# CycloneBoy/pdf_table

Hardware: AMD Instinct MI355X
Metric: pages/s (higher is better)
Workload: dtype bf16

## Files before the change

### include/pdftable_hip.h

```cpp
#ifndef PDFTABLE_HIP_H
#define PDFTABLE_HIP_H

#include <stddef.h>
#include <stdint.h>

#ifdef __cplusplus
extern "C" {
#endif

#define PT_OK 0
#define PT_ERR_INVALID 1
#define PT_ERR_HIP 2
#define PT_ERR_STATE 3
#define PT_ERR_FORMAT 4

typedef struct pt_engine pt_engine;
typedef void* pt_stream;

int pt_engine_create(int device_id, pt_engine** out);
void pt_engine_destroy(pt_engine* e);
const char* pt_last_error(void);
int pt_abi_version(void);
int pt_engine_check(pt_engine* e);
int pt_engine_set_lstm_cluster(pt_engine* e, int on);
// ... 162 lines not shown
                        const double* d_affine, int32_t* d_counts, float* d_cells, pt_stream stream);

int pt_tsr_process(pt_engine* e, const float* d_logi, const float* d_dets, const int32_t* h_counts, int n_tables,
                   int use_2dpe, float* d_logic, float* d_stacked, pt_stream stream);

int pt_op_conv2d(pt_engine* e, const uint16_t* d_in, int B, int H, int W, int Cin, const uint16_t* d_w_tiled,
                 const float* d_bias, int N, int ks, int stride, uint16_t* d_out, int out_cstride, int out_coff,
                 int rep, int shuffle_cout, const uint16_t* d_res, int res_mode, int relu, int split, int out_lo_off,
                 pt_stream stream);
int pt_op_conv1x1_ex(pt_engine* e, const uint16_t* d_in, int B, int H, int W, int Cin, const uint16_t* d_w_tiled, const float* d_bias,
                     int N, uint16_t* d_out, float* d_out_f32, int out_cstride, int n_valid, const float* d_res_f32, int relu,
                     const int32_t* d_ylimit, pt_stream stream);

int pt_op_dcn(pt_engine* e, const uint16_t* d_in, const float* d_om, int B, int H, int W, int C, const uint16_t* d_w_tiled,
              const float* d_bias, int N, uint16_t* d_out, int relu, int split, pt_stream stream);

int pt_op_stem7x7(pt_engine* e, const uint16_t* d_in, int B, int H, int W, const uint16_t* d_w, const float* d_bias,
                  uint16_t* d_out, int split, pt_stream stream);
int pt_op_maxpool3x3s2(pt_engine* e, const uint16_t* d_in, int B, int H, int W, int C, uint16_t* d_out, int split,
                       pt_stream stream);
int pt_op_db_head_final(pt_engine* e, const uint16_t* d_in, int B, int H, int W, const void* d_w, const float* d_bias,
                        float* d_prob, float* d_logits, int split, pt_stream stream);

int pt_op_dwconv(pt_engine* e, const uint16_t* d_in, int B, int H, int W, int C, const float* d_w_taps, const float* d_bias, int k,
                 int stride, int act, uint16_t* d_out, int split, pt_stream stream);
int pt_op_add(pt_engine* e, const uint16_t* d_a, const uint16_t* d_b, uint16_t* d_out, long long npix, int C, int split, pt_stream stream);
int pt_op_maxpool(pt_engine* e, const uint16_t* d_in, int B, int H, int W, int C, int k, int stride, int pad, uint16_t* d_out,
                  int split, pt_stream stream);
int pt_op_avgpool(pt_engine* e, const uint16_t* d_in, int B, int H, int W, int C, int k, uint16_t* d_out, int split, pt_stream stream);
int pt_op_chan_mean(pt_engine* e, const uint16_t* d_in, int B, int HW, int C, float* d_scratch, uint16_t* d_mean, int split, pt_stream stream);
// ... 90 lines not shown
```

### pdf_table_amd/csrc/c_api.hip

```cpp
#include <stdarg.h>
#include <stdio.h>
#include <stdlib.h>

#include <cmath>

#include "common.h"

namespace PT_FMT_NS {
namespace api {

static int ensure(void** buf, size_t* cap, size_t need);

int pt_engine_check(pt_engine* e) {
  PT_REQUIRE(e, "pt_engine_check: null engine");
  if (e->lstm_err && *e->lstm_err) {
    *e->lstm_err = 0;
    e->lstm_cluster = 0;
    pt_set_error("lstm_cluster_kernel: a workgroup waited > 2^22 polls for its peers -- the launch was not co-resident "
                 "(GPU shared with another process or stream?).  The recognition results since the last check are invalid; "
                 "this engine now uses the streaming LSTM kernel (pt_engine_set_lstm_cluster(e, 0)): run the batch again");
    return PT_ERR_HIP;
  }
  return PT_OK;
}
// ... 943 lines not shown
}

int pt_op_db_head_final(pt_engine* e, const uint16_t* d_in, int B, int H, int W, const void* d_w, const float* d_bias,
                        float* d_prob, float* d_logits, int split, pt_stream stream) {
  PT_REQUIRE(e && d_in && d_w && d_bias && (d_prob || d_logits), "pt_op_db_head_final: bad arguments");
  return pt_launch_db_head_final(d_in, B, H, W, d_w, d_bias, d_prob, d_logits, split, reinterpret_cast<hipStream_t>(stream));
}

int pt_op_dcn(pt_engine* e, const uint16_t* d_in, const float* d_om, int B, int H, int W, int C, const uint16_t* d_w_tiled,
              const float* d_bias, int N, uint16_t* d_out, int relu, int split, pt_stream stream) {
  PT_REQUIRE(e && d_in && d_om && d_w_tiled && d_bias && d_out, "pt_op_dcn: null argument");
  PT_REQUIRE(B > 0 && H > 0 && W > 0, "pt_op_dcn: empty map (B=%d H=%d W=%d)", B, H, W);
  return pt_launch_dcn_fused(e, d_in, d_om, d_w_tiled, d_bias, d_out, B, H, W, C, N, split, relu, reinterpret_cast<hipStream_t>(stream));
}

int pt_profile_enable(pt_engine* e, int on) {
  PT_REQUIRE(e != nullptr, "pt_profile_enable: null engine");
  PT_REQUIRE(on >= 0 && on < 2 + PT_PROF_NCLASS, "pt_profile_enable: mode %d out of range", on);
  if (on && !e->prof.h_lims)
    PT_HIP_CHECK(hipHostMalloc(reinterpret_cast<void**>(&e->prof.h_lims), PtProfile::MAX_LIMS * sizeof(int), hipHostMallocDefault));
  e->prof.on = on;
  return PT_OK;
}

int pt_profile_read_labels(pt_engine* e, char* buf, int cap) {
  PT_REQUIRE(e && buf && cap > 0, "pt_profile_read_labels: bad arguments");
  PT_HIP_CHECK(hipDeviceSynchronize());
  struct Row { double ms = 0, flop = 0, bytes = 0; long long n = 0; };
  std::map<std::string, Row> rows;
  for (auto& p : e->prof.pending) {
// ... 69 lines not shown
```

### pdf_table_amd/csrc/common.h

```cpp
#pragma once
#include <hip/hip_runtime.h>
#include <stdint.h>
#include <string.h>

#include <map>
#include <string>
#include <vector>

#include "../../include/pdftable_hip.h"
#include "act16.h"

typedef uint16_t bf16_t;

void pt_set_error(const char* fmt, ...);

#define PT_HIP_CHECK(expr)                                                                  \
  do {                                                                                      \
    hipError_t _e = (expr);                                                                 \
    if (_e != hipSuccess) {                                                                 \
      pt_set_error("%s failed: %s (%s:%d)", #expr, hipGetErrorString(_e), __FILE__, __LINE__); \
      return PT_ERR_HIP;                                                                    \
    }                                                                                       \
  } while (0)

// ... 219 lines not shown
  int alg_n = 0;
  double alg_scale = 1.0;
};
int pt_launch_conv(pt_engine* e, const ConvDesc& d, hipStream_t s);
int pt_launch_crnn_conv01(pt_engine* e, const bf16_t* gray, int n, const float* w64x9, const float* b0, const bf16_t* w1, const float* b1, bf16_t* p1,
                          const int* xlimit, const int* xlimit_cols, hipStream_t s);
int pt_launch_dwpw(pt_engine* e, const bf16_t* in, int B, int H, int W, int C, const float* dw_w, const float* dw_b, int k, int stride, int dw_act,
                   const ConvDesc& pw, hipStream_t s);

int pt_launch_stem7x7(pt_engine* e, const bf16_t* in, int B, int H, int W, const bf16_t* w, const float* bias,
                      bf16_t* out, int split, hipStream_t s, int stride = 2, int n_valid = 0);

int pt_launch_det_preprocess(const uint8_t* pages, int n, int h, int w, int nh, int nw, int flavour, int split,
                             bf16_t* out, hipStream_t s);
int pt_launch_dcn_fused(pt_engine* e, const bf16_t* x, const float* om, const bf16_t* w, const float* bias, bf16_t* out,
                        int B, int H, int W, int C, int N, int split, int relu, hipStream_t s, const bf16_t* omw = nullptr, const float* omb = nullptr);
bool pt_dcn_fuses_om(const pt_engine* e, int C, int split);
int pt_launch_maxpool3x3s2(const bf16_t* in, int B, int H, int W, int C, bf16_t* out, int split, hipStream_t s);
int pt_launch_stem7x7_pool(pt_engine* e, const bf16_t* in, int B, int H, int W, const bf16_t* w, const float* bias, bf16_t* out,
                           hipStream_t s);
int pt_launch_db_head_final(const bf16_t* in, int B, int H, int W, const void* w4x64, const float* bias, float* prob,
                            float* logits, int split, hipStream_t s);
int pt_launch_db_head_mfma(const bf16_t* in, int B, int H, int W, const bf16_t* w3, const float* b3, const bf16_t* w6,
                           const float* b6, float* prob, float* logits, hipStream_t s, uint32_t* bitmap = nullptr, float thresh = 0.f);
int pt_launch_bitmap(const float* prob, int n, int H, int W, float thresh, int dilate, uint32_t* bitmap,
                     hipStream_t s);
int pt_launch_box_scores(const float* prob, int n, int H, int W, const float* boxes, int nb, float* scores,
                         hipStream_t s);

#define PT_SE_CHUNKS 64
int pt_launch_stem3x3s2(const bf16_t* in, const float* w, const float* b, bf16_t* out, int B, int H, int W, int split,
                        hipStream_t s, int variant);
// ... 144 lines not shown
```

### pdf_table_amd/csrc/dla_net.h

```cpp
#pragma once

#include <stdlib.h>

#include <string>
#include <vector>

#include "net_ctx.h"

namespace PT_FMT_NS {

int pt_launch_conv3x3_c16(pt_engine* e, const bf16_t* in, const bf16_t* w, const float* bias, bf16_t* out, int B, int H, int W,
                          int N, int stride, int split, hipStream_t s);
int pt_launch_dla_thin_chain(pt_engine* e, const bf16_t* in, int B, int H, int W, const bf16_t* w_stem, const float* b_stem, const bf16_t* w0,
                             const float* b0, const bf16_t* w1, const float* b1, bf16_t* out, hipStream_t s);

namespace {

struct DlaCtx : NetCtx {
  bf16_t* cols = nullptr;
  float* om = nullptr;
  const int* ylimit = nullptr;
  double alg_scale = 1.0;

  void conv(const T& in, const std::string& q, int N, int ks, int stride, const T& out, int relu, const T* res = nullptr,
// ... 31 lines not shown
      e->prof.next_bytes = (double)n * x.H * x.W * x.C * 2.0 * mul * 1.25;
      PtProfScope ps(e, s, PT_PROF_OTHER, 0, "maxpool2x2");
      const int r = pt_launch_maxpool_kxk(x.p, n, x.H, x.W, x.C, 2, 2, 0, x3, o.p, s);
      if (r != PT_OK) rc = r;
    }
    return o;
  }
  T block(const std::string& q, const T& x, const T& residual, int stride, int cout) {
    T t = alloc(x.H / stride, x.W / stride, cout);
    conv(x, q + ".conv1", cout, 3, stride, t, 1);
    T o = alloc(t.H, t.W, cout);
    conv(t, q + ".conv2", cout, 3, 1, o, 1, &residual);
    return o;
  }
  T tree(const std::string& q, int levels, const T& x, int cin, int cout, int stride, bool level_root,
         std::vector<T> children) {
    T bottom = stride > 1 ? maxpool2(x) : x;
    if (level_root) children.push_back(bottom);
    if (levels == 1) {
      T residual = bottom;
      if (cin != cout) {
        residual = alloc(bottom.H, bottom.W, cout);
        conv(bottom, q + ".project", cout, 1, 1, residual, 0);
      }
      T x1 = block(q + ".tree1", x, residual, stride, cout);
      T x2 = block(q + ".tree2", x1, x1, 1, cout);
      std::vector<T> ins = {x2, x1};
      ins.insert(ins.end(), children.begin(), children.end());
      T o = alloc(x1.H, x1.W, cout);
      conv_cat(ins, q + ".root", cout, o, 1);
      return o;
    }
    T x1 = tree(q + ".tree1", levels - 1, x, cin, cout, stride, false, {});
    children.push_back(x1);
    return tree(q + ".tree2", levels - 1, x1, cout, cout, 1, false, children);
  }
};

static std::vector<T> dla34_base(DlaCtx& c, const bf16_t* x, int H, int W) {
  pt_engine* e = c.e;
  hipStream_t s = c.s;
  const int n = c.n;
  const int ch[6] = {16, 32, 64, 128, 256, 512};
  const int lv[6] = {1, 1, 1, 2, 2, 1};
  const char* chain_env = getenv("PT_DLA_CHAIN");
  const bool chain = !c.x3 && H % 2 == 0 && W % 2 == 0 && !(chain_env && atoi(chain_env) == 0);
  std::vector<T> layers(6);
  if (chain) {
// ... 37 lines not shown
```

### pdf_table_amd/csrc/lore_kernels.hip

```cpp
#include <stdio.h>
#include <stdlib.h>

#include "common.h"

namespace PT_FMT_NS {

typedef __attribute__((ext_vector_type(4))) uint32_t u32x4;
typedef __attribute__((ext_vector_type(2))) uint32_t u32x2;

namespace {

__device__ __forceinline__ float bf2f(uint32_t b) { return a16_to_f32(b); }
__device__ __forceinline__ uint32_t f2bf(float f) { return f32_to_a16(f); }

__device__ __forceinline__ void load8(const bf16_t* p, int lo_off, int split, float* v) {
  const u32x4 h = *reinterpret_cast<const u32x4*>(p);
  const uint32_t hw[4] = {h.x, h.y, h.z, h.w};
#pragma unroll
  for (int k = 0; k < 8; ++k) v[k] = bf2f((k & 1) ? (hw[k >> 1] >> 16) : (hw[k >> 1] & 0xFFFFu));
  if (split) {
    const u32x4 l = *reinterpret_cast<const u32x4*>(p + lo_off);
    const uint32_t lw[4] = {l.x, l.y, l.z, l.w};
#pragma unroll
    for (int k = 0; k < 8; ++k) v[k] += bf2f((k & 1) ? (lw[k >> 1] >> 16) : (lw[k >> 1] & 0xFFFFu));
// ... 451 lines not shown
    for (int r = 0; r < 16; ++r) {
      const long long op = p0 + wave * 32 + (r & 3) + 8 * (r >> 2) + 4 * q;
      if (op >= npix) continue;
      float v = acc[t][r] + bv;
      if (relu) v = fmaxf(v, 0.f);
      const uint32_t hb = f2bf(v);
      out[(size_t)op * ocs + n] = (bf16_t)hb;
      if (SPLIT) out[(size_t)op * ocs + N + n] = (bf16_t)f2bf(v - bf2f(hb));
    }
  }
}

#ifndef PT_DCN_ABL
#define PT_DCN_ABL 0
#endif
template <int NB, int NTHR, int SPLIT = 0, int EARLY = 0, int OMF = 0>
__global__ __launch_bounds__(NTHR, SPLIT ? (NB == 128 ? 1 : 2) : NTHR / 128) void dcn_fused64_kernel(const bf16_t* __restrict__ x, const float* __restrict__ om,
                                                              const bf16_t* __restrict__ w, const float* __restrict__ bias,
                                                              bf16_t* __restrict__ out, long long npix, int H, int W,
                                                              int C, int N, int relu, const bf16_t* __restrict__ omw = nullptr,
                                                              const float* __restrict__ omb = nullptr) {
#pragma clang fp contract(fast)
  a16_kernel_enter();
  constexpr int ROW = 144;
  constexpr int IT = 1024 / NTHR;
  constexpr int PSTEP = NTHR / 8;
  constexpr int WP = NB * 8 / NTHR;
  constexpr int NT = NB * 8 / NTHR;
  constexpr int NP = SPLIT ? 2 : 1;
  __shared__ __attribute__((aligned(16))) unsigned s_goff[128 * 9][4];
  __shared__ __attribute__((aligned(16))) float s_gwt[128 * 9][4];
  __shared__ __attribute__((aligned(16))) char s_ab[NP * (128 * ROW + NB * ROW)];
  static_assert(128 * ROW + NB * ROW >= 128 * 28 * 4, "operand images must cover the staged offset/mask rows");
  constexpr int A_PLANE = 128 * ROW, W_PLANE = NB * ROW;
  char* s_a = s_ab;
  char* s_w = s_ab + NP * A_PLANE;
  float* s_om = reinterpret_cast<float*>(s_ab);
// ... 7 lines not shown
  const int ty0 = (Lb % tiles_y) * 8;
  const long long img0 = (long long)(Lb / tiles_y) * H * W;
  auto locate = [&](int pl, int& y, int& xq) -> bool {
    y = ty0 + (pl >> 4);
    xq = tx0 + (pl & 15);
    const bool ok = y < H && xq < W;
    y = y < H ? y : H - 1;
    xq = xq < W ? xq : W - 1;
    return ok;
  };
  const int n0 = nblk * NB;
  const int nss = C >> 6, nst = 9 * nss, nk = 9 * (C >> 5);
  const int cs = SPLIT ? 2 * C : C;
  const int piece = tid & 7, prow = tid >> 3;
  const char* xmap = reinterpret_cast<const char*>(x + (size_t)img0 * cs);
  if constexpr (OMF) {
    constexpr int HP = 180, HROW = 80;
    constexpr int HIT = (HP * 4 + NTHR - 1) / NTHR;
    constexpr int NG = NTHR / 256;
    static_assert(sizeof(s_goff) >= HP * HROW && sizeof(s_gwt) >= HP * HROW, "a halo buffer must fit each table's space");
    char* s_h = reinterpret_cast<char*>(&s_goff[0][0]);
    char* s_h2 = reinterpret_cast<char*>(&s_gwt[0][0]);
    const int nch = (SPLIT ? 3 : 1) * (C >> 5);
    const int grp = wave >> 2, mt_o = wave & 3;
    const int t_lo = NG == 2 ? (grp ? 5 : 0) : 0, t_hi = NG == 2 ? (grp ? 9 : 5) : 9;
    u32x4 hreg[HIT];
    auto halo_load = [&](int kc) {
      int c0 = kc * 32;
      if (SPLIT && kc >= 2 * (C >> 5)) c0 -= 2 * C;
#pragma unroll
// ... 269 lines not shown
        }
      }
      __syncthreads();
      product();
    }
  } else {
    prefetch(0);
    for (int st = 0; st < nst; ++st) {
      __syncthreads();
      commit();
      __syncthreads();
      if (st + 1 < nst) prefetch(st + 1);
      product();
    }
  }
  int y, xq;
  if (locate(mt * 32 + lx, y, xq)) {
    bf16_t* op = out + (size_t)(img0 + (long long)y * W + xq) * (SPLIT ? 2 * N : N) + n0 + ct0 * 32;
#pragma unroll
    for (int t = 0; t < NT; ++t)
#pragma unroll
      for (int rg = 0; rg < 4; ++rg) {
        const int ch = t * 32 + 8 * rg + 4 * q;
        const float4 bs = *reinterpret_cast<const float4*>(bias + n0 + ct0 * 32 + ch);
        float v[4] = {acc[t][rg * 4 + 0] + bs.x, acc[t][rg * 4 + 1] + bs.y, acc[t][rg * 4 + 2] + bs.z, acc[t][rg * 4 + 3] + bs.w};
        if (relu) {
#pragma unroll
          for (int j = 0; j < 4; ++j) v[j] = fmaxf(v[j], 0.f);
        }
        const uint32_t h0 = f2bf(v[0]), h1 = f2bf(v[1]), h2 = f2bf(v[2]), h3 = f2bf(v[3]);
        *reinterpret_cast<uint2*>(op + ch) = make_uint2(h0 | (h1 << 16), h2 | (h3 << 16));
        if (SPLIT)
          *reinterpret_cast<uint2*>(op + N + ch) = make_uint2(f2bf(v[0] - bf2f(h0)) | (f2bf(v[1] - bf2f(h1)) << 16),
                                                               f2bf(v[2] - bf2f(h2)) | (f2bf(v[3] - bf2f(h3)) << 16));
      }
  }
}

#ifndef PT_DCN_MABL
#define PT_DCN_MABL 0
#endif
#ifndef PT_DCN_RING64
#define PT_DCN_RING64 4
#endif
template <int NB, int RING>
// ... 884 lines not shown
  PT_HIP_CHECK(hipGetLastError());
  return PT_OK;
}

bool pt_dcn_fuses_om(const pt_engine* e, int C, int split) {
  const char* ev = getenv("PT_DCN_FUSE_OM");
  const int on = ev ? atoi(ev) : 1;
  const char* nt = getenv("PT_DCN_THREADS");
  const char* ea = getenv("PT_DCN_EARLY");
  const char* xf = getenv("PT_DCN_X3_FAST");
  const bool defaults = !(nt && atoi(nt) != 512) && !(ea && atoi(ea) == 0) && !(xf && atoi(xf) == 0);
  if (!on || !e || C % 64 != 0 || !defaults || (!split && e->dcn_mfma != 0)) return false;
  return on == 2 || (!split && C <= 128);
}

int pt_launch_dcn_fused(pt_engine* e, const bf16_t* x, const float* om, const bf16_t* w, const float* bias, bf16_t* out,
                        int B, int H, int W, int C, int N, int split, int relu, hipStream_t s, const bf16_t* omw, const float* omb) {
  PT_REQUIRE(e && x && (om || (omw && omb)) && w && bias && out && C % 32 == 0 && N % 64 == 0, "dcn fused: bad arguments (C=%d N=%d)", C, N);
  PT_REQUIRE(!omw || pt_dcn_fuses_om(e, C, split), "dcn fused: the offset conv can only be fused on the default fused64 paths (C=%d)", C);
  PT_REQUIRE((long long)H * W * (split ? 2 * C : C) < (1ll << 31), "dcn fused: image too large for 32-bit offsets");
  const double dcn_bytes = (double)B * H * W * ((split ? 2.0 : 1.0) * 2.0 * (C + N) + 27 * 4.0) + (double)N * 9 * C * 2.0 * (split ? 3 : 1);
  e->prof.next_bytes = dcn_bytes;
  static int x3fast = -1;
  if (x3fast < 0) {
    const char* ev = getenv("PT_DCN_X3_FAST");
    x3fast = ev ? atoi(ev) : 1;
  }
  if (split && C % 64 == 0 && x3fast) {
    const long long npix = (long long)B * H * W;
    char label[48];
    snprintf(label, sizeof(label), "dcn fused %d->%d @%dx%d x3", C, N, H, W);
    PtProfScope prof(e, s, PT_PROF_OTHER, 0, label);
    const unsigned tiles = (unsigned)((long long)B * ((H + 7) / 8) * ((W + 15) / 16));
    const char* nbv = getenv("PT_DCN_NB");
    if (N % 128 == 0 && !(nbv && atoi(nbv) == 64)) {
      if (omw) hipLaunchKernelGGL((dcn_fused64_kernel<128, 512, 1, 0, 1>), dim3(tiles, N / 128), dim3(512), 0, s, x, om, w, bias, out, npix, H, W, C, N, relu, omw, omb);
      else hipLaunchKernelGGL((dcn_fused64_kernel<128, 512, 1>), dim3(tiles, N / 128), dim3(512), 0, s, x, om, w, bias, out, npix, H, W, C, N, relu, omw, omb);
    } else {
      if (omw) hipLaunchKernelGGL((dcn_fused64_kernel<64, 512, 1, 0, 1>), dim3(tiles, N / 64), dim3(512), 0, s, x, om, w, bias, out, npix, H, W, C, N, relu, omw, omb);
      else hipLaunchKernelGGL((dcn_fused64_kernel<64, 512, 1>), dim3(tiles, N / 64), dim3(512), 0, s, x, om, w, bias, out, npix, H, W, C, N, relu, omw, omb);
    }
    PT_HIP_CHECK(hipGetLastError());
    return PT_OK;
  }
  if (split) { e->prof.next_bytes = dcn_bytes; return launch_dcn_fused<1, 64>(e, x, om, w, bias, out, B, H, W, C, N, relu, s); }
  if (C % 64 == 0) {
    const long long npix = (long long)B * H * W;
    char label[48];
    snprintf(label, sizeof(label), "dcn fused %d->%d @%dx%d", C, N, H, W);
    PtProfScope prof(e, s, PT_PROF_OTHER, 0, label);
    static int nb128 = -1;
    if (nb128 < 0) {
      const char* ev = getenv("PT_DCN_NB");
      nb128 = ev ? (atoi(ev) == 128) : 1;
    }
    static int nthr = -1;
    if (nthr < 0) {
      const char* ev = getenv("PT_DCN_THREADS");
      nthr = ev ? atoi(ev) : 512;
    }
    const unsigned tiles = (unsigned)((long long)B * ((H + 7) / 8) * ((W + 15) / 16));
    static int mfma_nb = -1;
    if (mfma_nb < 0) {
      const char* nv = getenv("PT_DCN_MFMA_NB");
      PT_HIP_CHECK(hipFuncSetAttribute(reinterpret_cast<const void*>(&dcn_mfma_kernel<64, PT_DCN_RING64>), hipFuncAttributeMaxDynamicSharedMemorySize, DcnMfmaSmem<64, PT_DCN_RING64>::BYTES));
      PT_HIP_CHECK(hipFuncSetAttribute(reinterpret_cast<const void*>(&dcn_mfma_kernel<128, 8>), hipFuncAttributeMaxDynamicSharedMemorySize, DcnMfmaSmem<128, 8>::BYTES));
      mfma_nb = nv ? atoi(nv) : 128;
    }
    const int mfma = e->dcn_mfma;
    if (mfma == 2 && N == 64) {
      static bool attr2 = false;
      if (!attr2) {
        PT_HIP_CHECK(hipFuncSetAttribute(reinterpret_cast<const void*>(&dcn_mfma2_kernel), hipFuncAttributeMaxDynamicSharedMemorySize, DcnMfma2Smem::BYTES));
        attr2 = true;
      }
      const unsigned tiles2 = (unsigned)((long long)B * ((H + 15) / 16) * ((W + 15) / 16));
      hipLaunchKernelGGL(dcn_mfma2_kernel, dim3(tiles2, 1), dim3(512), DcnMfma2Smem::BYTES, s, x, om, w, bias, out, npix, H, W, C, N, relu);
      PT_HIP_CHECK(hipGetLastError());
      return PT_OK;
    }
    if (mfma == 1) {
      constexpr int smem64 = DcnMfmaSmem<64, PT_DCN_RING64>::BYTES, smem128 = DcnMfmaSmem<128, 8>::BYTES;
      if (N % 128 == 0 && mfma_nb == 128)
        hipLaunchKernelGGL((dcn_mfma_kernel<128, 8>), dim3(tiles, N / 128), dim3(512), smem128, s, x, om, w, bias, out, npix, H, W, C, N, relu);
// ... 79 lines not shown
```

### pdf_table_amd/csrc/lore_model.hip

```cpp
#include "dla_net.h"

namespace PT_FMT_NS {

int pt_launch_dcn_im2col(const bf16_t* x, const float* om, bf16_t* cols, int B, int H, int W, int C, int split,
                         hipStream_t s);
int pt_launch_dwconvt_up_add(const bf16_t* in, const float* w, const bf16_t* add, bf16_t* out, int B, int h, int wd,
                             int C, int f, int split, hipStream_t s);

namespace {

struct Ctx : DlaCtx {
  T dcn(const std::string& q, const T& x, int cout) {
    T o = alloc(x.H, x.W, cout);
    static const bool fused = !(getenv("PT_DCN_FUSED") && atoi(getenv("PT_DCN_FUSED")) == 0);
    const bool om_inside = fused && pt_dcn_fuses_om(e, x.C, x3);
    if (!om_inside) conv(x, q + ".om", 64, 3, 1, T(), 0, nullptr, 32, om, 32, 0, 27);
    if (fused) {
      const PtTensor* w = get(q + (x3 ? ".dcn.w3" : ".dcn.w"));
      const PtTensor* b = get(q + ".dcn.b");
      const PtTensor* ow = om_inside ? get(q + (x3 ? ".om.w3" : ".om.w")) : nullptr;
      const PtTensor* ob = om_inside ? get(q + ".om.b") : nullptr;
      if (go()) {
        const int r = pt_launch_dcn_fused(e, x.p, om, W(w), F(b), o.p, n, x.H, x.W, x.C, cout, x3, 1, s, ow ? W(ow) : nullptr, ob ? F(ob) : nullptr);
        if (r != PT_OK) rc = r;
      }
      return o;
    }
    if (go()) {
      PtProfScope ps(e, s, PT_PROF_OTHER, 0, "dcn im2col");
      const int r = pt_launch_dcn_im2col(x.p, om, cols, n, x.H, x.W, x.C, x3, s);
      if (r != PT_OK) rc = r;
    }
    T c;
    c.p = cols; c.H = x.H; c.W = x.W; c.C = 9 * x.C;
    conv(c, q + ".dcn", cout, 1, 1, o, 1);
    return o;
  }
  void ida(const std::string& q, std::vector<T>& layers, int startp, int endp, int o_ch, const int* up_f) {
    for (int i = startp + 1; i < endp; ++i) {
      const int j = i - startp;
      const std::string js = std::to_string(j);
      T p = dcn(q + ".proj_" + js, layers[i], o_ch);
      const int f = up_f[j];
      T u = alloc(p.H * f, p.W * f, o_ch);
      const PtTensor* wu = get(q + ".up_" + js + ".wf32");
      if (go()) {
        e->prof.next_bytes = (double)n * p.H * p.W * o_ch * 2.0 * mul * (1.0 + 2.0 * f * f);
        char label[48];
        snprintf(label, sizeof(label), "dw convT up + add %d @%dx%d", o_ch, p.H * f, p.W * f);
        PtProfScope ps(e, s, PT_PROF_OTHER, 0, label);
        const int r = pt_launch_dwconvt_up_add(p.p, F(wu), layers[i - 1].p, u.p, n, p.H, p.W, o_ch, f, x3, s);
        if (r != PT_OK) rc = r;
      }
      layers[i] = dcn(q + ".node_" + js, u, o_ch);
    }
  }
};

}

struct SparseArgs {
  int wiz_rev;
  float vis_thresh;
  int* d_counts;
  float *d_dets, *d_logi;
};

static int lore_dla_run(pt_engine* e, const bf16_t* x, int n, int H, int W, float* hm, float* st, float* wh, float* ax,
                        float* cr, float* reg, const SparseArgs* sp, hipStream_t s) {
// ... 9 lines not shown
  const int hreal[6] = {2, 8, 8, 256, 256, 2};

  return pt_plan_then_launch(c, "Lore net", [&]() -> int {
    const size_t px4 = (size_t)n * (H / 4) * (W / 4);
    c.cols = c.take<bf16_t>(px4 * 576 * c.mul * sizeof(bf16_t));
    c.om = c.take<float>(px4 * 32 * sizeof(float));

    std::vector<T> layers = dla34_base(c, x, H, W);

    std::vector<T> out = {layers[5]};
    const int f2[4] = {1, 2, 2, 2};
    c.ida("dla_up.ida_0", layers, 4, 6, 256, f2);
    out.insert(out.begin(), layers[5]);
    c.ida("dla_up.ida_1", layers, 3, 6, 128, f2);
    out.insert(out.begin(), layers[5]);
    c.ida("dla_up.ida_2", layers, 2, 6, 64, f2);
    out.insert(out.begin(), layers[5]);
    std::vector<T> y = {out[0], out[1], out[2]};
    const int f24[3] = {1, 2, 4};
    c.ida("ida_up", y, 0, 3, 64, f24);
    const T feat = y[2];
    T hid = c.alloc(feat.H, feat.W, 256);
    if (sp) heads[0] = c.take<float>((size_t)n * feat.H * feat.W * 8 * sizeof(float));
    for (int h = 0; h < 6; ++h) {
      if (sp && h != 0) continue;
      c.conv(feat, std::string(hname[h]) + ".0", 256, 3, 1, hid, 1);
      c.conv(hid, std::string(hname[h]) + ".2", hcs[h] < 64 ? 64 : hcs[h], 1, 1, T(), 0, nullptr, hcs[h], heads[h], hcs[h], 0, hreal[h]);
    }
    if (sp) {
      int rows_ax = 0, rows_cr = 0, rows_cell = 0, rows_corner = 0;
      pt_lore_mosaic_rows(n, &rows_ax, &rows_cr, &rows_cell, &rows_corner);
      const int MW = 32;
      auto mosaic = [&](int rows, int C) {
        T t;
        t.H = rows; t.W = MW; t.C = C;
// ... 153 lines not shown
```

### pdf_table_amd/engine.py

```python
from __future__ import annotations

import contextlib
import ctypes as C
import functools
import threading
from typing import Optional, Sequence, Tuple

import numpy as np
import torch

from . import lib as L

__all__ = ["HipEngine", "REC_LINE_DTYPE", "CLS_IMAGE_DTYPE", "REC_PP_ITEM_DTYPE"]

TSR_TABLE_DTYPE = np.dtype([("minv", "<f8", (6,)), ("page", "<i4"), ("x0", "<i4"), ("y0", "<i4"),
                            ("crop_w", "<i4"), ("crop_h", "<i4"), ("reserved", "<i4")])
CLS_IMAGE_DTYPE = np.dtype([("offset", "<i8"), ("h", "<i4"), ("w", "<i4")])
REC_LINE_DTYPE = np.dtype([("minv", np.float64, (9,)), ("page", np.int32), ("crop_w", np.int32), ("crop_h", np.int32),
                           ("reserved", np.int32)])


REC_PP_ITEM_DTYPE = np.dtype([("line", "<i4"), ("resized_w", "<i4"), ("img_w", "<i4"), ("reserved", "<i4"),
                              ("out_off", "<i8")])

# ... 629 lines not shown
    def op_dcn(self, x: torch.Tensor, om: torch.Tensor, w_tiled: torch.Tensor, bias: torch.Tensor, relu: bool = True, split: int = 0) -> torch.Tensor:
        self._chk(x, self.act_dtype, "x")
        self._chk(om, torch.float32, "om")
        self._chk(bias, torch.float32, "bias")
        B, H, W, Cc = x.shape
        m = 2 if split else 1
        Cc //= m
        if tuple(om.shape) != (B, H, W, 32):
            raise ValueError(f"op_dcn: om must be [B,H,W,32], got {tuple(om.shape)}")
        N = bias.numel()
        out = torch.empty((B, H, W, N * m), dtype=self.act_dtype, device=self._tdev)
        L.check(self.lib.pt_op_dcn(self._h, _ptr(x), _ptr(om), B, H, W, Cc, _ptr(w_tiled), _ptr(bias), N, _ptr(out), int(relu), int(split),
                                   self._stream()), "pt_op_dcn")
        return out

    def op_dwconv(self, x: torch.Tensor, w_taps: torch.Tensor, bias: torch.Tensor, k: int, stride: int = 1, act: int = 0, split: bool = False) -> torch.Tensor:
        self._chk(x, self.act_dtype, "x")
        self._chk(w_taps, torch.float32, "w_taps")
        self._chk(bias, torch.float32, "bias")
        B, H, W, Cc = x.shape
        pad = k // 2
        out = torch.empty((B, (H + 2 * pad - k) // stride + 1, (W + 2 * pad - k) // stride + 1, Cc), dtype=self.act_dtype, device=self._tdev)
        L.check(self.lib.pt_op_dwconv(self._h, _ptr(x), B, H, W, Cc // 2 if split else Cc, _ptr(w_taps), _ptr(bias), k, stride, act, _ptr(out), int(split),
                                      self._stream()), "pt_op_dwconv")
        return out

    def op_add(self, a: torch.Tensor, b: torch.Tensor, split: bool = False) -> torch.Tensor:
        self._chk(a, self.act_dtype, "a")
        self._chk(b, self.act_dtype, "b")
        if a.shape != b.shape:
# ... 332 lines not shown
```

### pdf_table_amd/lib.py

```python
from __future__ import annotations

import ctypes as C
import os

_HERE = os.path.dirname(os.path.abspath(__file__))
LIB_PATH = os.environ.get("PT_LIB_PATH") or os.path.join(_HERE, "libpdftable_hip.so")

PT_MODEL_DB_RESNET18 = 1
PT_MODEL_CRNN = 2
PT_MODEL_LORE_DLA34 = 3
PT_MODEL_LORE_PROCESSOR = 4
PT_MODEL_PICODET = 5
PT_MODEL_LORE_RESNET18 = 6
PT_MODEL_DB_NAS = 7
PT_MODEL_PPLCNET = 8
PT_MODEL_CONVNEXT_VIT = 16
PT_MODEL_MTL_BACKBONE = 17
PT_MODEL_MTL_DECODER = 18
PT_MODEL_CENTERNET_DLA34 = 19
PT_CVIT_W, PT_CVIT_CHUNK_W, PT_CVIT_CHUNK_STEP, PT_CVIT_T, PT_CVIT_NCLS = 804, 300, 252, 201, 7644
PT_CLS_SLOTS = 4
PT_CLS_MAX_CLASSES = 16
PT_LAYOUT_HEAD_CS, PT_LAYOUT_CAND_FLOATS = 40, 48
PT_DET_PRE_DB_PP = 0
# ... 75 lines not shown
        "pt_centernet_decode": (i, [vp, vp, vp, vp, vp, i, i, i, vp, vp, vp, vp]),
        "pt_hard_nms": (i, [vp, vp, vp, i, C.c_double, i, vp, vp]),
        "pt_page_line_mask": (i, [vp, i, i, i, vp, vp]),
        "pt_page_line_angles": (i, [vp, i, i, i, i, i, vp, i, vp]),
        "pt_page_warp_cubic": (i, [vp, i, i, i, vp, vp, i, vp, vp]),
        "pt_page_quarter_turn": (i, [vp, i, i, i, i, vp, vp]),
        "pt_page_pre_tables": (i, [vp, vp]),
        "pt_cls_preprocess": (i, [vp, vp, vp, i, i, i, i, i, vp, vp]),
        "pt_cls_forward_net": (i, [vp, i, vp, i, i, i, i, vp, ip, vp]),
        "pt_cls_forward": (i, [vp, i, vp, vp, i, i, i, i, i, i, vp, ip, vp]),
        "pt_cls_forward_lines": (i, [vp, i, vp, i, i, i, vp, vp, i, i, i, i, i, i, vp, ip, vp]),
        "pt_cls_forward_lines_direct": (i, [vp, i, vp, i, i, i, vp, i, i, i, i, i, i, vp, ip, vp]),
        "pt_op_conv2d": (i, [vp, vp, i, i, i, i, vp, vp, i, i, i, vp, i, i, i, i, vp, i, i, i, i, vp]),
        "pt_op_conv1x1_ex": (i, [vp, vp, i, i, i, i, vp, vp, i, vp, vp, i, i, vp, i, vp, vp]),
        "pt_op_dcn": (i, [vp, vp, vp, i, i, i, i, vp, vp, i, vp, i, i, vp]),
        "pt_op_stem7x7": (i, [vp, vp, i, i, i, vp, vp, vp, i, vp]),
        "pt_op_maxpool3x3s2": (i, [vp, vp, i, i, i, i, vp, i, vp]),
        "pt_op_db_head_final": (i, [vp, vp, i, i, i, vp, vp, vp, vp, i, vp]),
        "pt_op_dwconv": (i, [vp, vp, i, i, i, i, vp, vp, i, i, i, vp, i, vp]),
        "pt_op_add": (i, [vp, vp, vp, vp, C.c_longlong, i, i, vp]),
        "pt_op_maxpool": (i, [vp, vp, i, i, i, i, i, i, i, vp, i, vp]),
        "pt_op_avgpool": (i, [vp, vp, i, i, i, i, i, vp, i, vp]),
        "pt_op_chan_mean": (i, [vp, vp, i, i, i, vp, vp, i, vp]),
        "pt_op_chan_mean_scratch_floats": (i, [i, i]),
        "pt_op_scale_channels": (i, [vp, vp, vp, i, i, i, vp, i, vp]),
        "pt_op_act": (i, [vp, vp, C.c_longlong, i, C.c_float, C.c_float, vp, i, i, vp]),
        "pt_op_copy_channels": (i, [vp, vp, C.c_longlong, i, i, vp, i, i, i, vp]),
        "pt_op_upsample_nearest": (i, [vp, vp, i, i, i, i, i, vp, vp]),
        "pt_op_mul": (i, [vp, vp, vp, vp, C.c_longlong, i, i, vp]),
        "pt_copy_bytes": (i, [vp, vp, vp, C.c_longlong, vp]),
# ... 49 lines not shown
```

Before: 804.4.

## Fuse depthwise transposed-conv upsample+add into DCN node epilogue; pool once in DLA tree

Adds an epilogue to the fused DCN kernel that stages the low-resolution projection patch and the transposed-conv taps in dead shared buffers. The kernel then computes the 2x/4x depthwise upsample and adds it to the node output, so the separate dwconvT up+add launch and its full-resolution read and write go away. The IDA aggregation is reordered so each node's DCN emits the next level's upsampled sum directly. The change also reuses the pooled input in DLA tree recursion instead of max-pooling twice. It costs extra shared memory, registers and epilogue work in the DCN kernel, and is limited to the default single-pass configurations.

```diff
diff --git a/include/pdftable_hip.h b/include/pdftable_hip.h
--- a/include/pdftable_hip.h
+++ b/include/pdftable_hip.h
@@ -200,6 +200,12 @@
 
 int pt_op_dcn(pt_engine* e, const uint16_t* d_in, const float* d_om, int B, int H, int W, int C, const uint16_t* d_w_tiled,
               const float* d_bias, int N, uint16_t* d_out, int relu, int split, pt_stream stream);
+
+int pt_op_dwconvt_up_add(pt_engine* e, const uint16_t* d_in, const float* d_w, const uint16_t* d_add, uint16_t* d_out, int B, int h, int w, int C,
+                         int f, int split, pt_stream stream);
+int pt_op_dcn_up_add(pt_engine* e, const uint16_t* d_in, const float* d_om, int B, int H, int W, int C, const uint16_t* d_w_tiled,
+                     const float* d_bias, int N, uint16_t* d_out, int relu, int split, const uint16_t* d_up_in, int up_h, int up_w,
+                     const float* d_up_w, int up_f, pt_stream stream);
 
 int pt_op_stem7x7(pt_engine* e, const uint16_t* d_in, int B, int H, int W, const uint16_t* d_w, const float* d_bias,
                   uint16_t* d_out, int split, pt_stream stream);
diff --git a/pdf_table_amd/csrc/c_api.hip b/pdf_table_amd/csrc/c_api.hip
--- a/pdf_table_amd/csrc/c_api.hip
+++ b/pdf_table_amd/csrc/c_api.hip
@@ -981,6 +981,25 @@
   return pt_launch_dcn_fused(e, d_in, d_om, d_w_tiled, d_bias, d_out, B, H, W, C, N, split, relu, reinterpret_cast<hipStream_t>(stream));
 }
 
+int pt_op_dwconvt_up_add(pt_engine* e, const uint16_t* d_in, const float* d_w, const uint16_t* d_add, uint16_t* d_out, int B, int h, int w, int C,
+                         int f, int split, pt_stream stream) {
+  PT_REQUIRE(e && d_in && d_w && d_out, "pt_op_dwconvt_up_add: null argument");
+  PT_REQUIRE(B > 0 && h > 0 && w > 0 && C > 0, "pt_op_dwconvt_up_add: empty map (B=%d h=%d w=%d C=%d)", B, h, w, C);
+  return pt_launch_dwconvt_up_add(d_in, d_w, d_add, d_out, B, h, w, C, f, split, reinterpret_cast<hipStream_t>(stream));
+}
+
+int pt_op_dcn_up_add(pt_engine* e, const uint16_t* d_in, const float* d_om, int B, int H, int W, int C, const uint16_t* d_w_tiled,
+                     const float* d_bias, int N, uint16_t* d_out, int relu, int split, const uint16_t* d_up_in, int up_h, int up_w,
+                     const float* d_up_w, int up_f, pt_stream stream) {
+  PT_REQUIRE(e && d_in && d_om && d_w_tiled && d_bias && d_out && d_up_in && d_up_w, "pt_op_dcn_up_add: null argument");
+  PT_REQUIRE(B > 0 && H > 0 && W > 0, "pt_op_dcn_up_add: empty map (B=%d H=%d W=%d)", B, H, W);
+  PT_REQUIRE(split == 0, "pt_op_dcn_up_add: the (hi | lo) modes keep the two launches (pt_op_dcn, pt_op_dwconvt_up_add)");
+  PT_REQUIRE((up_f == 2 || up_f == 4) && up_h > 0 && up_w > 0 && up_h * up_f == H && up_w * up_f == W,
+             "pt_op_dcn_up_add: a %dx%d map times %d is not the %dx%d output", up_h, up_w, up_f, H, W);
+  return pt_launch_dcn_fused(e, d_in, d_om, d_w_tiled, d_bias, d_out, B, H, W, C, N, split, relu, reinterpret_cast<hipStream_t>(stream), nullptr, nullptr,
+                             d_up_in, d_up_w, up_f);
+}
+
 int pt_profile_enable(pt_engine* e, int on) {
   PT_REQUIRE(e != nullptr, "pt_profile_enable: null engine");
   PT_REQUIRE(on >= 0 && on < 2 + PT_PROF_NCLASS, "pt_profile_enable: mode %d out of range", on);
diff --git a/pdf_table_amd/csrc/common.h b/pdf_table_amd/csrc/common.h
--- a/pdf_table_amd/csrc/common.h
+++ b/pdf_table_amd/csrc/common.h
@@ -257,8 +257,12 @@
 int pt_launch_det_preprocess(const uint8_t* pages, int n, int h, int w, int nh, int nw, int flavour, int split,
                              bf16_t* out, hipStream_t s);
 int pt_launch_dcn_fused(pt_engine* e, const bf16_t* x, const float* om, const bf16_t* w, const float* bias, bf16_t* out,
-                        int B, int H, int W, int C, int N, int split, int relu, hipStream_t s, const bf16_t* omw = nullptr, const float* omb = nullptr);
+                        int B, int H, int W, int C, int N, int split, int relu, hipStream_t s, const bf16_t* omw = nullptr, const float* omb = nullptr,
+                        const bf16_t* up_in = nullptr, const float* up_w = nullptr, int up_f = 0);
 bool pt_dcn_fuses_om(const pt_engine* e, int C, int split);
+bool pt_dcn_fuses_up(const pt_engine* e, int C, int N, int split);
+int pt_launch_dwconvt_up_add(const bf16_t* in, const float* w, const bf16_t* add, bf16_t* out, int B, int h, int wd, int C, int f, int split,
+                             hipStream_t s);
 int pt_launch_maxpool3x3s2(const bf16_t* in, int B, int H, int W, int C, bf16_t* out, int split, hipStream_t s);
 int pt_launch_stem7x7_pool(pt_engine* e, const bf16_t* in, int B, int H, int W, const bf16_t* w, const float* bias, bf16_t* out,
                            hipStream_t s);
diff --git a/pdf_table_amd/csrc/dla_net.h b/pdf_table_amd/csrc/dla_net.h
--- a/pdf_table_amd/csrc/dla_net.h
+++ b/pdf_table_amd/csrc/dla_net.h
@@ -69,8 +69,8 @@
     return o;
   }
   T tree(const std::string& q, int levels, const T& x, int cin, int cout, int stride, bool level_root,
-         std::vector<T> children) {
-    T bottom = stride > 1 ? maxpool2(x) : x;
+         std::vector<T> children, const T* pooled = nullptr) {
+    T bottom = stride > 1 ? (pooled ? *pooled : maxpool2(x)) : x;
     if (level_root) children.push_back(bottom);
     if (levels == 1) {
       T residual = bottom;
@@ -86,7 +86,9 @@
       conv_cat(ins, q + ".root", cout, o, 1);
       return o;
     }
-    T x1 = tree(q + ".tree1", levels - 1, x, cin, cout, stride, false, {});
+    const char* once_env = getenv("PT_DLA_POOL_ONCE");
+    const bool once = stride > 1 && !(once_env && atoi(once_env) == 0);
+    T x1 = tree(q + ".tree1", levels - 1, x, cin, cout, stride, false, {}, once ? &bottom : nullptr);
     children.push_back(x1);
     return tree(q + ".tree2", levels - 1, x1, cout, cout, 1, false, children);
   }
diff --git a/pdf_table_amd/csrc/lore_kernels.hip b/pdf_table_amd/csrc/lore_kernels.hip
--- a/pdf_table_amd/csrc/lore_kernels.hip
+++ b/pdf_table_amd/csrc/lore_kernels.hip
@@ -489,13 +489,17 @@
 #ifndef PT_DCN_ABL
 #define PT_DCN_ABL 0
 #endif
-template <int NB, int NTHR, int SPLIT = 0, int EARLY = 0, int OMF = 0>
+__device__ __forceinline__ float dcn_up_mad(float acc, float v, float wt) { return acc + v * wt; }
+
+template <int NB, int NTHR, int SPLIT = 0, int EARLY = 0, int OMF = 0, int UPF = 0>
 __global__ __launch_bounds__(NTHR, SPLIT ? (NB == 128 ? 1 : 2) : NTHR / 128) void dcn_fused64_kernel(const bf16_t* __restrict__ x, const float* __restrict__ om,
                                                               const bf16_t* __restrict__ w, const float* __restrict__ bias,
                                                               bf16_t* __restrict__ out, long long npix, int H, int W,
                                                               int C, int N, int relu, const bf16_t* __restrict__ omw = nullptr,
-                                                              const float* __restrict__ omb = nullptr) {
+                                                              const float* __restrict__ omb = nullptr, const bf16_t* __restrict__ up_in = nullptr,
+                                                              const float* __restrict__ up_w = nullptr) {
 #pragma clang fp contract(fast)
+  static_assert(UPF == 0 || ((UPF == 2 || UPF == 4) && !SPLIT), "the up-sampling epilogue exists for factors 2 and 4 of the single-pass modes");
   a16_kernel_enter();
   constexpr int ROW = 144;
   constexpr int IT = 1024 / NTHR;
@@ -533,6 +537,25 @@
   const int cs = SPLIT ? 2 * C : C;
   const int piece = tid & 7, prow = tid >> 3;
   const char* xmap = reinterpret_cast<const char*>(x + (size_t)img0 * cs);
+  constexpr int UPH = UPF ? 8 / UPF + 2 : 1, UPW = UPF ? 16 / UPF + 2 : 1;
+  constexpr int UPITCH = NB * 2 + 16, WPITCH = NB + 8;
+  constexpr int UPP = UPF ? (UPH * UPW * (NB / 8) + NTHR - 1) / NTHR : 1;
+  constexpr int UPWT = UPF ? (4 * UPF * UPF * (NB / 4) + NTHR - 1) / NTHR : 1;
+  [[maybe_unused]] u32x4 upreg[UPP];
+  if constexpr (UPF != 0) {
+    static_assert(UPH * UPW * UPITCH <= (int)sizeof(s_ab) && 4 * UPF * UPF * WPITCH * 4 <= (int)sizeof(s_gwt), "the staged patch and table must fit the dead buffers");
+    const int uh = H / UPF, uw = W / UPF;
+    const long long ub = (img0 / ((long long)H * W)) * uh;
+#pragma unroll
+    for (int j = 0; j < UPP; ++j) {
+      const int i = tid + j * NTHR, pp = i / (NB / 8), pc = i - pp * (NB / 8);
+      const int r = pp / UPW, c = pp - r * UPW;
+      const int iy = min(max(ty0 / UPF - 1 + r, 0), uh - 1), ix = min(max(tx0 / UPF - 1 + c, 0), uw - 1);
+      u32x4 v = {0u, 0u, 0u, 0u};
+      if (i < UPH * UPW * (NB / 8)) v = *reinterpret_cast<const u32x4*>(up_in + (size_t)((ub + iy) * uw + ix) * N + n0 + pc * 8);
+      upreg[j] = v;
+    }
+  }
   if constexpr (OMF) {
     constexpr int HP = 180, HROW = 80;
     constexpr int HIT = (HP * 4 + NTHR - 1) / NTHR;
@@ -832,9 +855,49 @@
       product();
     }
   }
+  if constexpr (UPF != 0) {
+    float4 wreg[UPWT];
+#pragma unroll
+    for (int j = 0; j < UPWT; ++j) {
+      const int i = tid + j * NTHR;
+      float4 v = make_float4(0.f, 0.f, 0.f, 0.f);
+      if (i < 4 * UPF * UPF * (NB / 4)) v = *reinterpret_cast<const float4*>(up_w + (size_t)(i / (NB / 4)) * N + n0 + (i % (NB / 4)) * 4);
+      wreg[j] = v;
+    }
+    __syncthreads();
+#pragma unroll
+    for (int j = 0; j < UPP; ++j) {
+      const int i = tid + j * NTHR, pp = i / (NB / 8), pc = i - pp * (NB / 8);
+      if (i < UPH * UPW * (NB / 8)) *reinterpret_cast<u32x4*>(s_ab + pp * UPITCH + pc * 16) = upreg[j];
+    }
+#pragma unroll
+    for (int j = 0; j < UPWT; ++j) {
+      const int i = tid + j * NTHR;
+      if (i < 4 * UPF * UPF * (NB / 4)) *reinterpret_cast<float4*>(reinterpret_cast<float*>(&s_gwt[0][0]) + (i / (NB / 4)) * WPITCH + (i % (NB / 4)) * 4) = wreg[j];
+    }
+    __syncthreads();
+  }
   int y, xq;
   if (locate(mt * 32 + lx, y, xq)) {
     bf16_t* op = out + (size_t)(img0 + (long long)y * W + xq) * (SPLIT ? 2 * N : N) + n0 + ct0 * 32;
+    [[maybe_unused]] const char* up_p[2][2];
+    [[maybe_unused]] const float* up_t[2][2];
+    [[maybe_unused]] bool up_ok[2][2];
+    if constexpr (UPF != 0) {
+      const int uh = H / UPF, uw = W / UPF;
+      const int iy1 = (y + UPF / 2) / UPF, ix1 = (xq + UPF / 2) / UPF;
+#pragma unroll
+      for (int dy = 0; dy < 2; ++dy)
+#pragma unroll
+        for (int dx = 0; dx < 2; ++dx) {
+          const int iy = iy1 - dy, ix = ix1 - dx;
+          const int ky = y + UPF / 2 - iy * UPF, kx = xq + UPF / 2 - ix * UPF;
+          up_ok[dy][dx] = iy >= 0 && iy < uh && ix >= 0 && ix < uw;
+          const int iyc = min(max(iy, 0), uh - 1), ixc = min(max(ix, 0), uw - 1);
+          up_p[dy][dx] = s_ab + ((iyc - (ty0 / UPF - 1)) * UPW + (ixc - (tx0 / UPF - 1))) * UPITCH + ct0 * 64;
+          up_t[dy][dx] = reinterpret_cast<const float*>(&s_gwt[0][0]) + (ky * (2 * UPF) + kx) * WPITCH + ct0 * 32;
+        }
+    }
 #pragma unroll
     for (int t = 0; t < NT; ++t)
 #pragma unroll
@@ -846,7 +909,24 @@
 #pragma unroll
           for (int j = 0; j < 4; ++j) v[j] = fmaxf(v[j], 0.f);
         }
-        const uint32_t h0 = f2bf(v[0]), h1 = f2bf(v[1]), h2 = f2bf(v[2]), h3 = f2bf(v[3]);
+        uint32_t h0 = f2bf(v[0]), h1 = f2bf(v[1]), h2 = f2bf(v[2]), h3 = f2bf(v[3]);
+        if constexpr (UPF != 0) {
+          float us[4] = {0.f, 0.f, 0.f, 0.f};
+#pragma unroll
+          for (int dy = 0; dy < 2; ++dy)
+#pragma unroll
+            for (int dx = 0; dx < 2; ++dx) {
+              if (UPF == 4 && !up_ok[dy][dx]) continue;
+              uint2 pv = *reinterpret_cast<const uint2*>(up_p[dy][dx] + ch * 2);
+              if (UPF == 2 && !up_ok[dy][dx]) pv = make_uint2(0u, 0u);
+              const float4 wv = *reinterpret_cast<const float4*>(up_t[dy][dx] + ch);
+              us[0] = dcn_up_mad(us[0], bf2f(pv.x & 0xFFFFu), wv.x);
+              us[1] = dcn_up_mad(us[1], bf2f(pv.x >> 16), wv.y);
+              us[2] = dcn_up_mad(us[2], bf2f(pv.y & 0xFFFFu), wv.z);
+              us[3] = dcn_up_mad(us[3], bf2f(pv.y >> 16), wv.w);
+            }
+          h0 = f2bf(us[0] + bf2f(h0)); h1 = f2bf(us[1] + bf2f(h1)); h2 = f2bf(us[2] + bf2f(h2)); h3 = f2bf(us[3] + bf2f(h3));
+        }
         *reinterpret_cast<uint2*>(op + ch) = make_uint2(h0 | (h1 << 16), h2 | (h3 << 16));
         if (SPLIT)
           *reinterpret_cast<uint2*>(op + N + ch) = make_uint2(f2bf(v[0] - bf2f(h0)) | (f2bf(v[1] - bf2f(h1)) << 16),
@@ -1761,12 +1841,27 @@
   return on == 2 || (!split && C <= 128);
 }
 
+bool pt_dcn_fuses_up(const pt_engine* e, int C, int N, int split) {
+  const char* ev = getenv("PT_IDA_FUSE_UP");
+  if ((ev && atoi(ev) == 0) || !e || split || e->dcn_mfma != 0 || C != N || (N != 64 && N != 128)) return false;
+  for (const char* name : {"PT_DCN_FUSED", "PT_DCN_FUSE_OM", "PT_DCN_THREADS", "PT_DCN_EARLY", "PT_DCN_NB", "PT_DCN_MFMA", "PT_DCN_MFMA_NB", "PT_DCN_X3_FAST"})
+    if (getenv(name)) return false;
+  return true;
+}
+
 int pt_launch_dcn_fused(pt_engine* e, const bf16_t* x, const float* om, const bf16_t* w, const float* bias, bf16_t* out,
-                        int B, int H, int W, int C, int N, int split, int relu, hipStream_t s, const bf16_t* omw, const float* omb) {
+                        int B, int H, int W, int C, int N, int split, int relu, hipStream_t s, const bf16_t* omw, const float* omb,
+                        const bf16_t* up_in, const float* up_w, int up_f) {
   PT_REQUIRE(e && x && (om || (omw && omb)) && w && bias && out && C % 32 == 0 && N % 64 == 0, "dcn fused: bad arguments (C=%d N=%d)", C, N);
   PT_REQUIRE(!omw || pt_dcn_fuses_om(e, C, split), "dcn fused: the offset conv can only be fused on the default fused64 paths (C=%d)", C);
   PT_REQUIRE((long long)H * W * (split ? 2 * C : C) < (1ll << 31), "dcn fused: image too large for 32-bit offsets");
-  const double dcn_bytes = (double)B * H * W * ((split ? 2.0 : 1.0) * 2.0 * (C + N) + 27 * 4.0) + (double)N * 9 * C * 2.0 * (split ? 3 : 1);
+  if (up_f) {
+    PT_REQUIRE(up_in && up_w && (up_f == 2 || (up_f == 4 && N == 64)) && H % up_f == 0 && W % up_f == 0,
+               "dcn fused + up: factor %d must be 2 (or 4 at 64 channels) and divide the %dx%d map", up_f, H, W);
+    PT_REQUIRE(pt_dcn_fuses_up(e, C, N, split), "dcn fused + up: only the default single-pass kernels at C = N = 64 or 128 carry the up-sampling epilogue (C=%d N=%d split=%d)", C, N, split);
+  }
+  const double dcn_bytes = (double)B * H * W * ((split ? 2.0 : 1.0) * 2.0 * (C + N) + 27 * 4.0) + (double)N * 9 * C * 2.0 * (split ? 3 : 1) +
+                           (up_f ? (double)B * (H / up_f) * (W / up_f) * N * 2.0 : 0.0);
   e->prof.next_bytes = dcn_bytes;
   static int x3fast = -1;
   if (x3fast < 0) {
@@ -1794,7 +1889,7 @@
   if (C % 64 == 0) {
     const long long npix = (long long)B * H * W;
     char label[48];
-    snprintf(label, sizeof(label), "dcn fused %d->%d @%dx%d", C, N, H, W);
+    snprintf(label, sizeof(label), "dcn fused%s %d->%d @%dx%d", up_f ? "+up" : "", C, N, H, W);
     PtProfScope prof(e, s, PT_PROF_OTHER, 0, label);
     static int nb128 = -1;
     if (nb128 < 0) {
@@ -1815,6 +1910,18 @@
       mfma_nb = nv ? atoi(nv) : 128;
     }
     const int mfma = e->dcn_mfma;
+    if (up_f) {
+      const unsigned blk = N == 128 ? 256 : 512;
+#define PT_DCN_UP(NB_, NT_, EARLY_, OMF_, UPF_)                                                                                                   \
+  hipLaunchKernelGGL((dcn_fused64_kernel<NB_, NT_, 0, EARLY_, OMF_, UPF_>), dim3(tiles, N / NB_), dim3(blk), 0, s, x, om, w, bias, out, npix, H, W, C, N, relu, \
+                     omw, omb, up_in, up_w)
+      if (N == 128) { if (omw) PT_DCN_UP(128, 256, 0, 1, 2); else PT_DCN_UP(128, 256, 0, 0, 2); }
+      else if (up_f == 2) { if (omw) PT_DCN_UP(64, 512, 1, 1, 2); else PT_DCN_UP(64, 512, 1, 0, 2); }
+      else { if (omw) PT_DCN_UP(64, 512, 1, 1, 4); else PT_DCN_UP(64, 512, 1, 0, 4); }
+#undef PT_DCN_UP
+      PT_HIP_CHECK(hipGetLastError());
+      return PT_OK;
+    }
     if (mfma == 2 && N == 64) {
       static bool attr2 = false;
       if (!attr2) {
diff --git a/pdf_table_amd/csrc/lore_model.hip b/pdf_table_amd/csrc/lore_model.hip
--- a/pdf_table_amd/csrc/lore_model.hip
+++ b/pdf_table_amd/csrc/lore_model.hip
@@ -4,13 +4,15 @@
 
 int pt_launch_dcn_im2col(const bf16_t* x, const float* om, bf16_t* cols, int B, int H, int W, int C, int split,
                          hipStream_t s);
-int pt_launch_dwconvt_up_add(const bf16_t* in, const float* w, const bf16_t* add, bf16_t* out, int B, int h, int wd,
-                             int C, int f, int split, hipStream_t s);
-
 namespace {
 
 struct Ctx : DlaCtx {
-  T dcn(const std::string& q, const T& x, int cout) {
+  struct UpTail {
+    T p;
+    const PtTensor* w = nullptr;
+    int f = 0;
+  };
+  T dcn(const std::string& q, const T& x, int cout, const UpTail* up = nullptr) {
     T o = alloc(x.H, x.W, cout);
     static const bool fused = !(getenv("PT_DCN_FUSED") && atoi(getenv("PT_DCN_FUSED")) == 0);
     const bool om_inside = fused && pt_dcn_fuses_om(e, x.C, x3);
@@ -21,7 +23,8 @@
       const PtTensor* ow = om_inside ? get(q + (x3 ? ".om.w3" : ".om.w")) : nullptr;
       const PtTensor* ob = om_inside ? get(q + ".om.b") : nullptr;
       if (go()) {
-        const int r = pt_launch_dcn_fused(e, x.p, om, W(w), F(b), o.p, n, x.H, x.W, x.C, cout, x3, 1, s, ow ? W(ow) : nullptr, ob ? F(ob) : nullptr);
+        const int r = pt_launch_dcn_fused(e, x.p, om, W(w), F(b), o.p, n, x.H, x.W, x.C, cout, x3, 1, s, ow ? W(ow) : nullptr, ob ? F(ob) : nullptr,
+                                          up ? up->p.p : nullptr, up ? F(up->w) : nullptr, up ? up->f : 0);
         if (r != PT_OK) rc = r;
       }
       return o;
@@ -36,23 +39,42 @@
     conv(c, q + ".dcn", cout, 1, 1, o, 1);
     return o;
   }
-  void ida(const std::string& q, std::vector<T>& layers, int startp, int endp, int o_ch, const int* up_f) {
+  void ida(const std::string& q, std::vector<T>& layers, int startp, int endp, int o_ch, const int* up_f, bool own_nodes = false,
+           const UpTail* tail = nullptr, const T* first_sum = nullptr) {
+    const bool fuse = own_nodes && pt_dcn_fuses_up(e, o_ch, o_ch, x3);
+    T p, u;
+    bool have_p = false, have_u = false;
+    if (first_sum) { u = *first_sum; have_p = have_u = true; }
     for (int i = startp + 1; i < endp; ++i) {
       const int j = i - startp;
       const std::string js = std::to_string(j);
-      T p = dcn(q + ".proj_" + js, layers[i], o_ch);
-      const int f = up_f[j];
-      T u = alloc(p.H * f, p.W * f, o_ch);
-      const PtTensor* wu = get(q + ".up_" + js + ".wf32");
-      if (go()) {
-        e->prof.next_bytes = (double)n * p.H * p.W * o_ch * 2.0 * mul * (1.0 + 2.0 * f * f);
-        char label[48];
-        snprintf(label, sizeof(label), "dw convT up + add %d @%dx%d", o_ch, p.H * f, p.W * f);
-        PtProfScope ps(e, s, PT_PROF_OTHER, 0, label);
-        const int r = pt_launch_dwconvt_up_add(p.p, F(wu), layers[i - 1].p, u.p, n, p.H, p.W, o_ch, f, x3, s);
-        if (r != PT_OK) rc = r;
-      }
-      layers[i] = dcn(q + ".node_" + js, u, o_ch);
+      if (!have_p) p = dcn(q + ".proj_" + js, layers[i], o_ch);
+      if (!have_u) {
+        const int f = up_f[j];
+        u = alloc(p.H * f, p.W * f, o_ch);
+        const PtTensor* wu = get(q + ".up_" + js + ".wf32");
+        if (go()) {
+          e->prof.next_bytes = (double)n * p.H * p.W * o_ch * 2.0 * mul * (1.0 + 2.0 * f * f);
+          char label[48];
+          snprintf(label, sizeof(label), "dw convT up + add %d @%dx%d", o_ch, p.H * f, p.W * f);
+          PtProfScope ps(e, s, PT_PROF_OTHER, 0, label);
+          const int r = pt_launch_dwconvt_up_add(p.p, F(wu), layers[i - 1].p, u.p, n, p.H, p.W, o_ch, f, x3, s);
+          if (r != PT_OK) rc = r;
+        }
+      }
+      have_p = have_u = false;
+      UpTail nx;
+      if (fuse && i + 1 < endp) {
+        const std::string ns = std::to_string(j + 1);
+        p = nx.p = dcn(q + ".proj_" + ns, layers[i + 1], o_ch);
+        nx.w = get(q + ".up_" + ns + ".wf32");
+        nx.f = up_f[j + 1];
+        have_p = true;
+      } else if (fuse && tail) {
+        nx = *tail;
+      }
+      layers[i] = dcn(q + ".node_" + js, u, o_ch, nx.f ? &nx : nullptr);
+      if (nx.f) { u = layers[i]; have_u = true; }
     }
   }
 };
@@ -92,11 +114,17 @@
     out.insert(out.begin(), layers[5]);
     c.ida("dla_up.ida_1", layers, 3, 6, 128, f2);
     out.insert(out.begin(), layers[5]);
-    c.ida("dla_up.ida_2", layers, 2, 6, 64, f2);
+    const int f24[3] = {1, 2, 4};
+    Ctx::UpTail t2;
+    if (pt_dcn_fuses_up(e, 64, 64, c.x3)) {
+      t2.p = c.dcn("ida_up.proj_1", out[0], 64);
+      t2.w = c.get("ida_up.up_1.wf32");
+      t2.f = f24[1];
+    }
+    c.ida("dla_up.ida_2", layers, 2, 6, 64, f2, true, t2.f ? &t2 : nullptr);
     out.insert(out.begin(), layers[5]);
     std::vector<T> y = {out[0], out[1], out[2]};
-    const int f24[3] = {1, 2, 4};
-    c.ida("ida_up", y, 0, 3, 64, f24);
+    c.ida("ida_up", y, 0, 3, 64, f24, true, nullptr, t2.f ? &y[0] : nullptr);
     const T feat = y[2];
     T hid = c.alloc(feat.H, feat.W, 256);
     if (sp) heads[0] = c.take<float>((size_t)n * feat.H * feat.W * 8 * sizeof(float));
diff --git a/pdf_table_amd/engine.py b/pdf_table_amd/engine.py
--- a/pdf_table_amd/engine.py
+++ b/pdf_table_amd/engine.py
@@ -667,6 +667,38 @@
                                    self._stream()), "pt_op_dcn")
         return out
 
+    def op_dwconvt_up_add(self, x: torch.Tensor, w_taps: torch.Tensor, add: Optional[torch.Tensor], f: int, split: int = 0) -> torch.Tensor:
+        self._chk(x, self.act_dtype, "x")
+        self._chk(w_taps, torch.float32, "w_taps")
+        B, h, w, Cc = x.shape
+        if add is not None:
+            self._chk(add, self.act_dtype, "add")
+            if tuple(add.shape) != (B, h * f, w * f, Cc):
+                raise ValueError(f"op_dwconvt_up_add: add must be {(B, h * f, w * f, Cc)}, got {tuple(add.shape)}")
+        out = torch.empty((B, h * f, w * f, Cc), dtype=self.act_dtype, device=self._tdev)
+        L.check(self.lib.pt_op_dwconvt_up_add(self._h, _ptr(x), _ptr(w_taps), _ptr(add), _ptr(out), B, h, w, Cc // 2 if split else Cc, int(f),
+                                              int(split), self._stream()), "pt_op_dwconvt_up_add")
+        return out
+
+    def op_dcn_up_add(self, x: torch.Tensor, om: torch.Tensor, w_tiled: torch.Tensor, bias: torch.Tensor, up_in: torch.Tensor, up_taps: torch.Tensor,
+                      f: int, relu: bool = True, split: int = 0) -> torch.Tensor:
+        self._chk(x, self.act_dtype, "x")
+        self._chk(om, torch.float32, "om")
+        self._chk(bias, torch.float32, "bias")
+        self._chk(up_in, self.act_dtype, "up_in")
+        self._chk(up_taps, torch.float32, "up_taps")
+        B, H, W, Cc = x.shape
+        if tuple(om.shape) != (B, H, W, 32):
+            raise ValueError(f"op_dcn_up_add: om must be [B,H,W,32], got {tuple(om.shape)}")
+        N = bias.numel()
+        if up_in.dim() != 4 or up_in.shape[0] != B or up_in.shape[3] != N:
+            raise ValueError(f"op_dcn_up_add: up_in must be [{B},h,w,{N}], got {tuple(up_in.shape)}")
+        out = torch.empty((B, H, W, N), dtype=self.act_dtype, device=self._tdev)
+        L.check(self.lib.pt_op_dcn_up_add(self._h, _ptr(x), _ptr(om), B, H, W, Cc // 2 if split else Cc, _ptr(w_tiled), _ptr(bias), N, _ptr(out), int(relu),
+                                          int(split), _ptr(up_in), up_in.shape[1], up_in.shape[2], _ptr(up_taps), int(f), self._stream()),
+                "pt_op_dcn_up_add")
+        return out
+
     def op_dwconv(self, x: torch.Tensor, w_taps: torch.Tensor, bias: torch.Tensor, k: int, stride: int = 1, act: int = 0, split: bool = False) -> torch.Tensor:
         self._chk(x, self.act_dtype, "x")
         self._chk(w_taps, torch.float32, "w_taps")
diff --git a/pdf_table_amd/lib.py b/pdf_table_amd/lib.py
--- a/pdf_table_amd/lib.py
+++ b/pdf_table_amd/lib.py
@@ -113,6 +113,8 @@
         "pt_op_conv2d": (i, [vp, vp, i, i, i, i, vp, vp, i, i, i, vp, i, i, i, i, vp, i, i, i, i, vp]),
         "pt_op_conv1x1_ex": (i, [vp, vp, i, i, i, i, vp, vp, i, vp, vp, i, i, vp, i, vp, vp]),
         "pt_op_dcn": (i, [vp, vp, vp, i, i, i, i, vp, vp, i, vp, i, i, vp]),
+        "pt_op_dwconvt_up_add": (i, [vp, vp, vp, vp, vp, i, i, i, i, i, i, vp]),
+        "pt_op_dcn_up_add": (i, [vp, vp, vp, i, i, i, i, vp, vp, i, vp, i, i, vp, i, i, vp, i, vp]),
         "pt_op_stem7x7": (i, [vp, vp, i, i, i, vp, vp, vp, i, vp]),
         "pt_op_maxpool3x3s2": (i, [vp, vp, i, i, i, i, vp, i, vp]),
         "pt_op_db_head_final": (i, [vp, vp, i, i, i, vp, vp, vp, vp, i, vp]),
```

Result: faster. 819.9 (median of 6 runs) (+1.9%).
